# Aedelon/ProteinBERT-PyTorch-Replication

Measured on AMD Instinct MI355X. Metric: sequences/sec (whole node) ProteinBERT pretrain L=512 at 1/2/4/8 MI355X, higher is better.
Workload: dtype bf16; 1 GPU; global_batch=2048, per_gpu_batch=2048, seq_len=512, parallelism=dp1, impl=hip, hip_graph=False

## Files before the change

### proteinbert_pytorch_replication_amd/ops/fused_model.py

```python
from __future__ import annotations

from typing import Dict, Tuple

import torch
import torch.nn.functional as F

from .global_track import FusedGlobalBlockFn, GlobalBlockFn, HeadsLossFn, InputLayerFn, glob_fused_ok, pack_batch
from . import local_track as _lt
from .local_track import CH, EmbedFn, conv_images, embed_tokens, local_block, wgrad_tok_ok
from .paper_track import PaperHeadsLossFn, paper_block, unit_attention_weight


def hip_supported(model) -> Tuple[bool, str]:
    cfg = model.config
    if cfg["local_dim"] != CH:
        return False, f"local_dim={cfg['local_dim']} (HIP kernels are specialised for 128)"
    if cfg["conv_kernel_size"] != 9:
        return False, f"conv_kernel_size={cfg['conv_kernel_size']} (HIP kernels are specialised for 9)"
    if cfg["vocab_size"] > 32:
        return False, "vocab_size > 32"
    if cfg["semantics"] == "paper":
        from .paper_attention import KEY_DIM, VALUE_DIM
        if cfg["key_dim"] != KEY_DIM or cfg["global_dim"] // cfg["num_heads"] != VALUE_DIM:
            return False, (f"paper semantics: the HIP attention core is built for key_dim={KEY_DIM}, "
                           f"value_dim={VALUE_DIM}")
    if (cfg["global_dim"] % 32) != 0:
        return False, "global_dim must be a multiple of 32"
    return True, ""


def _check(model) -> None:
    ok, why = hip_supported(model)
    if not ok:
        raise NotImplementedError(f"HIP backend: unsupported configuration: {why}")


def fused_encode(model, tokens: torch.Tensor, annotations: torch.Tensor,
                 return_bf16: bool = False, cp=None):
    _check(model)
    if cp is None:
        model.check_length(tokens.shape[1])
    else:
        model.check_length(cp.L)
        if tokens.shape[1] != cp.shard_len:
            raise ValueError(f"expected a {cp.shard_len}-residue shard, got {tokens.shape[1]}")
    blocks = list(model.proteinBERT_blocks)
    lin = model.global_linear_layer[0]
    gl0 = blocks[0].global_to_local_linear_layer[0]
    g, g_bf, gb = InputLayerFn.apply(annotations, lin.weight, lin.bias, gl0.weight, gl0.bias)
    paper = model.semantics == "paper"
    emb_w = model.local_embedding.weight
    tok_c = tokens.contiguous()
    fold = (_lt.EMBED_FOLD and cp is None and tokens.device.type == "cuda" and len(blocks) > 0
            and wgrad_tok_ok(tok_c, emb_w, tokens.shape[1], blocks[0].local_narrow_conv_layer[0].weight.shape[2]))
    if fold and not paper and _lt.EMBED_GATHER:
        h = None
    else:
        h = embed_tokens(tok_c, emb_w) if fold else EmbedFn.apply(tokens, emb_w)
    mask = (tokens != 0).contiguous() if paper else None
    items, conv_imgs, glob_imgs = [], [], []
    for i, blk in enumerate(blocks):
        imgs, it = conv_images(blk.local_narrow_conv_layer[0].weight, blk.local_wide_conv_layer[0].weight)
        conv_imgs.append(imgs)
        items += it
        nxt = blocks[i + 1].global_to_local_linear_layer[0] if i + 1 < len(blocks) else None
        if glob_fused_ok(g.shape[1], 0 if nxt is None else nxt.weight.shape[0]):
            ws = [blk.global_linear_layer_1[0].weight, blk.global_linear_layer_2[0].weight,
                  None if nxt is None else nxt.weight]
            imgs = []
            for w in ws:
                if w is None:
                    imgs += [None, None]
                    continue
                o1, o2 = (torch.empty(w.numel(), dtype=torch.bfloat16, device=w.device) for _ in range(2))
                imgs += [o1, o2]
                items.append((1, w.detach(), o1, o2, w.shape[0], w.shape[1]))
            glob_imgs.append(tuple(imgs))
        else:
            glob_imgs.append(None)
    pack_batch(items)
    for i, blk in enumerate(blocks):
        att = blk.global_attention_layer
        if paper:
            first = i == 0 and cp is None
            h, o = paper_block(h, gb, g, blk, mask, conv_imgs[i], tok=tok_c if first else None,
                               emb=emb_w if first else None, emb_grad=fold and i == 0, cp=cp)
            vpart = o.unsqueeze(1)
            wp = unit_attention_weight(att.key_dim, h.device)
        else:
            first = i == 0 and cp is None
            h, vpart = local_block(h, gb, blk, conv_imgs[i], tail=(i == 0), cp=cp,
                                   tok=tok_c if first else None, emb=emb_w if first else None,
                                   emb_grad=fold and i == 0)
            if cp is not None:
                vpart = cp.pool_sum(vpart)
            wp = att.W_parameter
        nxt = blocks[i + 1].global_to_local_linear_layer[0] if i + 1 < len(blocks) else None
        l1, l2 = blk.global_linear_layer_1[0], blk.global_linear_layer_2[0]
        n1, n2 = blk.global_norm_1, blk.global_norm_2
        args = (g, g_bf, vpart, l1.weight, l1.bias, n1.weight, n1.bias, l2.weight, l2.bias, n2.weight, n2.bias,
                wp, None if nxt is None else nxt.weight, None if nxt is None else nxt.bias)
        if glob_imgs[i] is not None:
            g, g_bf, gb = FusedGlobalBlockFn.apply(*args, glob_imgs[i])
        else:
            g, g_bf, gb = GlobalBlockFn.apply(*args)
    if return_bf16:
        return h, g, g_bf
    return h, g


def fused_forward(model, tokens: torch.Tensor, annotations: torch.Tensor):
    h, g = fused_encode(model, tokens, annotations)
    return model.heads_torch(h, g)


def fused_pretrain_loss(model, X: Dict[str, torch.Tensor], Y: Dict[str, torch.Tensor], W: Dict[str, torch.Tensor],
                        return_parts: bool = False, cp=None):
    h, g, g_bf = fused_encode(model, X["local"], X["global"], return_bf16=True, cp=cp)
    if cp is not None:
        W = dict(W, local=W["local"].float() * (cp.shard_len / cp.L))
    lo, go = model.pretraining_local_output[0], model.pretraining_global_output[0]
    fn = PaperHeadsLossFn if model.semantics == "paper" else HeadsLossFn
    total, parts = fn.apply(h, g, g_bf, lo.weight, lo.bias, go.weight, go.bias, Y["local"], Y["global"],
                                     W["local"], W["global"])
    if return_parts:
        return total, parts[0], parts[1]
    return total
```

### proteinbert_pytorch_replication_amd/ops/local_track.py

```python
from __future__ import annotations

import ctypes
import os
from typing import List, Dict, Optional, Tuple

import torch

from . import _lib, streams
from ..train.arena import notify_grads_ready
from ..utils.determinism import fused_deterministic
from .global_track import bf16_of

_P, _I, _F, _L = ctypes.c_void_p, ctypes.c_int, ctypes.c_float, ctypes.c_long

_lib.register("pbx_conv_fwd3x", [_P, _P, _P, _P, _P, _P, _P, _P, _P, _P, _I, _I, _I, _I, _I, _I, _P])
_lib.register("pbx_conv_fwd5x", [_P, _P, _P, _P, _P, _P, _P, _P, _P, _P, _I, _I, _I, _I, _I, _I, _P])
_lib.register("pbx_conv_dgrad4x", [_P, _P, _P, _P, _P, _P, _P, _P, _I, _I, _I, _I, _I, _I, _P])
_lib.register("pbx_wgrad2x", [_P, _P, _P, _P, _P, _P, _P, _P, _P, _I, _I, _I, _I, _I, _I, _I, _P])
_lib.register("pbx_pack_conv_frag", [_P, _P, _P, _I, _P])
_lib.register("pbx_wgrad2", [_P, _P, _P, _P, _P, _P, _P, _P, _P, _I, _I, _I, _I, _I, _P])
_lib.register("pbx_wgrad_tok", [_P, _P, _P, _P, _P, _P, _P, _P, _P, _P, _I, _I, _I, _I, _P, _P, _P, _P, _P])
_lib.register("pbx_ln_linear_fwd", [_P, _P, _I, _I, _P, _P, _P, _P, _P, _P, _P, _I, _I, _F, _P])
_lib.register("pbx_pool_fwd", [_P, _P, _P, _P, _P, _P, _P, _I, _I, _I, _F, _P])
_lib.register("pbx_pool_bwd", [_P, _P, _P, _P, _P, _I, _P, _P, _P, _I, _I, _I, _P])
_lib.register("pbx_ln2_linear_bwd", [_P, _P, _P, _P, _I, _P, _P, _P, _P, _I, _I, _P, _P, _P, _P, _P, _P, _P, _P,
                                     _P, _P, _P, _P, _P, _I, _I, _F, _P, _I, _I, _I, _I, _P])
_lib.register("pbx_ln2_bwd_slab_rows", [_I, _I, _I])
_lib.register("pbx_colsum_add", [_P, _I, _I, _P, _P, _P])
_lib.register("pbx_colsum_add2", [_P, _I, _P, _P, _I, _P, _I, _P])
_lib.register("pbx_ln1_finalize", [_P, _P, _P, _I, _I, _P, _I, _P, _P, _P, _I, _I, _F, _I, _P])
_lib.register("pbx_embed_fwd", [_P, _P, _P, _L, _P])
_lib.register("pbx_embed_bwd", [_P, _P, _P, _L, _I, _P, _P])
_lib.register("pbx_conv_fwd3t", [_P, _P, _P, _P, _P, _P, _P, _P, _P, _P, _P, _I, _I, _I, _I, _P])
_lib.register("pbx_conv_dgrad4f", [_P, _P, _P, _I, _I, _P, _I, _P, _P, _P, _P, _P, _P, _P, _P, _P, _I, _I, _I, _I,
                                    _F, _P])
_lib.register("pbx_embed_dpre", [_P, _P, _P, _P, _P, _P, _P, _L, _I, _P, _P])
_lib.register("pbx_embed_bwd_groups", [_L])

CH = 128
PB = 32
LN_EPS = 1e-5


BM1 = 128
def attn_pool_supported(NJ: int) -> bool:
    return NJ in (256, 512)


def conv_tile(L: int) -> int:
    return BM1


def _p(t: Optional[torch.Tensor]):
    return None if t is None else t.data_ptr()


CONV_FWD5 = os.environ.get("PBX_CONV_FWD", "5") == "5"


def conv_dgrad_fin(dh1, s1, st1, T1, BM1, sums1, TS1, g1, gdn, gdw, wtn, wtw, dx, dpn, dpw, dgb, B, L, KS, dil,
                   stream):
    _lib.call("pbx_conv_dgrad4f", dh1.data_ptr(), s1.data_ptr(), st1.data_ptr(), T1, BM1, sums1.data_ptr(),
              TS1, g1.data_ptr(), gdn.data_ptr(), gdw.data_ptr(), wtn.data_ptr(), wtw.data_ptr(),
              dx.data_ptr(), dpn.data_ptr(), dpw.data_ptr(), dgb.data_ptr(), B, L, KS, dil, LN_EPS, stream)


def conv_fwd(x, wpn, wpw, bn, bw, gb, pre_n, pre_w, s1, stats, B, L, KS, dil, stream, xlo: int = 0,
             xhi: int = 0) -> None:
    name = "pbx_conv_fwd5x" if (CONV_FWD5 and KS == 9 and dil == 5) else "pbx_conv_fwd3x"
    _lib.call(name, x.data_ptr(), wpn.data_ptr(), wpw.data_ptr(), bn.data_ptr(), bw.data_ptr(),
              gb.data_ptr(), _p(pre_n), _p(pre_w), s1.data_ptr(), stats.data_ptr(), B, L, KS, dil, xlo, xhi, stream)


def conv_dgrad(ds1, pre_n, pre_w, wtn, wtw, dx, dpn, dpw, B, L, KS, dil, stream, ilo: int = 0, ihi: int = 0) -> None:
    _lib.call("pbx_conv_dgrad4x", ds1.data_ptr(), pre_n.data_ptr(), pre_w.data_ptr(), wtn.data_ptr(),
              wtw.data_ptr(), dx.data_ptr(), dpn.data_ptr(), dpw.data_ptr(), B, L, KS, dil, ilo, ihi, stream)


_DWL_SLAB: Dict[int, torch.Tensor] = {}


def dwl_slab(dev: torch.device) -> Tuple[Optional[int], int]:
    idx = dev.index if dev.index is not None else torch.cuda.current_device()
    s = _DWL_SLAB.get(idx)
    rows = 2 * _num_cus(dev)
    if s is None:
        s = torch.empty(rows * (CH * CH + CH), dtype=torch.float32, device=dev)
        _DWL_SLAB[idx] = s
    return s.data_ptr(), rows


def _num_cus(dev: torch.device) -> int:
    return torch.cuda.get_device_properties(dev).multi_processor_count


def pack_conv(w: torch.Tensor) -> Tuple[torch.Tensor, torch.Tensor]:
    KS = w.shape[2]
    wp = torch.empty((KS, CH, CH), dtype=torch.bfloat16, device=w.device)
    wt = torch.empty_like(wp)
    _lib.call("pbx_pack_conv_frag", w.detach().contiguous().data_ptr(), wp.data_ptr(), wt.data_ptr(), KS,
              _lib.stream_ptr(w.device))
    return wp, wt


def _grad_dst(p: torch.Tensor, shape) -> Tuple[torch.Tensor, bool]:
    g = getattr(p, "grad", None) if getattr(p, "_pbx_arena", False) else None
    if g is not None and g.is_contiguous() and g.dtype == torch.float32 and tuple(g.shape) == tuple(shape):
        return g, True
    return torch.zeros(shape, dtype=torch.float32, device=p.device), False


WGRAD_TAIL_FULL = True
LN2_LATE_FOLD = True
DGRAD_FIN = True
INPUT_BWD_EARLY = True


WGRAD_CU_EIGHTHS = 8


def _wgrad(dy0: torch.Tensor, dy1: Optional[torch.Tensor], x: torch.Tensor, KS: int, dil: int, nconv: int,
           B: int, L: int, outs, full_chip: bool = False, xlo: int = 0, xhi: int = 0):
    dev = x.device
    ntiles = B * ((L + 127) // 128)
    R = max(8, (WGRAD_CU_EIGHTHS * _num_cus(dev) // (16 * nconv)) // 8 * 8)
    if full_chip:
        R = max(8, (_num_cus(dev) // (2 * nconv)) // 8 * 8)
    R = min(R, ntiles)
    slab = torch.empty((R, nconv, KS, CH, CH), dtype=torch.float32, device=dev)
    bslab = torch.empty((R, nconv, CH), dtype=torch.float32, device=dev)
    (dw0, db0) = outs[0]
    (dw1, db1) = outs[1] if nconv > 1 else (None, None)
    if xlo or xhi:
        _lib.call("pbx_wgrad2x", dy0.data_ptr(), _p(dy1), x.data_ptr(), slab.data_ptr(), bslab.data_ptr(),
                  dw0.data_ptr(), _p(dw1), db0.data_ptr(), _p(db1), B, L, dil, nconv, R, xlo, xhi, _lib.stream_ptr(dev))
    else:
        _lib.call("pbx_wgrad2", dy0.data_ptr(), _p(dy1), x.data_ptr(), slab.data_ptr(), bslab.data_ptr(),
                  dw0.data_ptr(), _p(dw1), db0.data_ptr(), _p(db1), B, L, dil, nconv, R, _lib.stream_ptr(dev))
    return [slab, bslab]


WGRAD_TOK = True
EMBED_FOLD = True
EMBED_GATHER = True


def wgrad_tok_ok(tok: Optional[torch.Tensor], emb: Optional[torch.Tensor], L: int, KS: int) -> bool:
    return (WGRAD_TOK and tok is not None and emb is not None and KS == 9 and L % 2 == 0
            and emb.shape[0] <= 32 and emb.shape[1] == CH and tok.dtype == torch.int64 and tok.is_contiguous())


def _wgrad_tok(dy0: torch.Tensor, dy1: torch.Tensor, tok: torch.Tensor, emb: torch.Tensor, dil: int, B: int, L: int,
               outs, demb=None):
    dev = dy0.device
    V = emb.shape[0]
    R = _lib.lib().pbx_wgrad_tok_rows(B, L)
    slab = torch.empty((R, 2, 9, V, CH), dtype=torch.float32, device=dev)
    S = torch.empty((2, 9, V, CH), dtype=torch.float32, device=dev)
    e = emb.detach().float().contiguous()
    (dw0, db0), (dw1, db1) = outs
    w0 = w1 = dE = dEslab = None
    if demb is not None:
        w0, w1 = (w.detach().float().contiguous() for w in demb[:2])
        dE = demb[2]
        dEslab = torch.empty((2 * CH, V, CH), dtype=torch.float32, device=dev)
    _lib.call("pbx_wgrad_tok", tok.data_ptr(), dy0.data_ptr(), dy1.data_ptr(), e.data_ptr(), slab.data_ptr(),
              S.data_ptr(), dw0.data_ptr(), dw1.data_ptr(), db0.data_ptr(), db1.data_ptr(), B, L, dil, V,
              _p(w0), _p(w1), _p(dE), _p(dEslab), _lib.stream_ptr(dev))
    return [slab, S, e, w0, w1, dEslab]


def embed_fold_bwd(tok, emb, ds1, gdn, gdw, dpn, dpw, wn, ww, stream):
    B, L = tok.shape
    dE, direct = _grad_dst(emb, emb.shape)
    slab = None
    if fused_deterministic():
        slab = torch.empty((_lib.lib().pbx_embed_bwd_groups(B * L), emb.shape[0], CH), dtype=torch.float32,
                           device=ds1.device)
    _lib.call("pbx_embed_dpre", tok.data_ptr(), ds1.data_ptr(), gdn.data_ptr(), gdw.data_ptr(), dpn.data_ptr(),
              dpw.data_ptr(), dE.data_ptr(), B * L, emb.shape[0], _p(slab), stream)
    return (wn, ww, dE), direct


class LocalBlockFn(torch.autograd.Function):

    @staticmethod
    def forward(ctx, x, gb, wn, bn, ww, bw, g1, be1, wl, bl, g2, be2, wv_bf16, dil: int, packed=None,
                tail: bool = False, cp=None, tok=None, emb=None, emb_grad: bool = False):
        params = (wn, bn, ww, bw, g1, be1, wl, bl, g2, be2)
        ctx.cp = cp
        if cp is not None:
            g1, be1, g2, be2 = (cp.rows(t) for t in (g1, be1, g2, be2))
        if x is None:
            if not (emb_grad and tok is not None and emb is not None and cp is None):
                raise ValueError("x may be None only for the folded first block (emb_grad with tok / emb)")
            B, L = tok.shape
            xt = torch.empty((B, L, CH), dtype=torch.bfloat16, device=tok.device)
        else:
            B, L, C = x.shape
            assert C == CH and x.dtype == torch.bfloat16 and x.is_contiguous()
            xt = x
        NJ = wv_bf16.shape[0]
        if not attn_pool_supported(NJ):
            raise NotImplementedError(f"HIP attention pool: H * value_dim = {NJ} (kernels built for 256 / 512)")
        KS = wn.shape[2]
        dev = xt.device
        stream = _lib.stream_ptr(dev)
        T1 = (L + BM1 - 1) // BM1
        T2 = (L + PB - 1) // PB
        if packed is not None:
            wpn, wtn, wpw, wtw = packed
        else:
            wpn, wtn = pack_conv(wn)
            wpw, wtw = pack_conv(ww)
        wl_b = bf16_of(wl)
        need_bwd = any(ctx.needs_input_grad)
        pre_n = torch.empty_like(xt) if need_bwd else None
        pre_w = torch.empty_like(xt) if need_bwd else None
        s1 = torch.empty_like(xt)
        st1 = torch.empty((B, T1, 2), dtype=torch.float32, device=dev)
        gb = gb.detach().float().contiguous()
        if x is None:
            x_ext, hlo = None, 0
            emb_b = bf16_of(emb)
            _lib.call("pbx_conv_fwd3t", tok.data_ptr(), emb_b.data_ptr(), wpn.data_ptr(), wpw.data_ptr(),
                      bn.data_ptr(), bw.data_ptr(), gb.data_ptr(), _p(pre_n), _p(pre_w), s1.data_ptr(),
                      st1.data_ptr(), B, L, KS, dil, stream)
        elif cp is None:
            x_ext, hlo = x, 0
            conv_fwd(x, wpn, wpw, bn, bw, gb, pre_n, pre_w, s1, st1, B, L, KS, dil, stream)
        else:
            x_ext, hlo = cp.halo_rows(x), cp.halo
            conv_fwd(x_ext, wpn, wpw, bn, bw, gb, pre_n, pre_w, s1, st1, B, L, KS, dil, stream, hlo, hlo)
            cp.fix_stats(st1, BM1)
        pre_l = torch.empty_like(xt) if need_bwd else None
        s2 = torch.empty_like(xt)
        st2 = torch.empty((B, T2, 2), dtype=torch.float32, device=dev)
        _lib.call("pbx_ln_linear_fwd", s1.data_ptr(), st1.data_ptr(), T1, BM1, g1.data_ptr(), be1.data_ptr(),
                  wl_b.data_ptr(), bl.data_ptr(), _p(pre_l), s2.data_ptr(), st2.data_ptr(), B, L, LN_EPS, stream)
        if cp is not None:
            cp.fix_stats(st2, PB)
        h2 = torch.empty_like(xt)
        TV = (L + 31) // 32
        vpart = torch.empty((B, TV, NJ), dtype=torch.float32, device=dev)
        _lib.call("pbx_pool_fwd", s2.data_ptr(), st2.data_ptr(), g2.data_ptr(), be2.data_ptr(), wv_bf16.data_ptr(),
                  h2.data_ptr(), vpart.data_ptr(), B, L, NJ, LN_EPS, stream)
        ctx.save_for_backward(x_ext, pre_n, pre_w, s1, st1, pre_l, s2, st2, h2, wtn, wtw, wl_b, wv_bf16, g1, be1, g2,
                              be2)
        ctx.hlo = hlo
        ctx.tok = (tok, emb) if cp is None and wgrad_tok_ok(tok, emb, L, KS) else None
        ctx.emb_grad = bool(emb_grad)
        if ctx.emb_grad and (ctx.tok is None or (x is not None and x.requires_grad)):
            raise ValueError("emb_grad needs a token-embedding input without autograd history (wgrad_tok_ok)")
        ctx.meta = (B, L, KS, dil, T1, T2, NJ)
        ctx.tail = bool(tail) and WGRAD_TAIL_FULL
        ctx.set_materialize_grads(False)
        ctx.params = params
        return h2, vpart

    @staticmethod
    def backward(ctx, dh2, dvpart):
        streams.wait_ready(dvpart, dh2)
        (x_ext, pre_n, pre_w, s1, st1, pre_l, s2, st2, h2, wtn, wtw, wl_b, wv_bf16, g1, be1, g2,
         be2) = ctx.saved_tensors
        cp, hlo = ctx.cp, ctx.hlo
        x = s1
        B, L, KS, dil, T1, T2, NJ = ctx.meta
        dev = x.device
        stream = _lib.stream_ptr(dev)
        params = ctx.params
        dsts = [_grad_dst(p, p.shape) for p in params]
        (dwn, _), (dbn, _), (dww, _), (dbw, _), (dg1, _), (dbe1, _), (dwl, _), (dbl, _), (dg2, _), (dbe2, _) = dsts
        if cp is not None:
            dg1, dbe1, dg2, dbe2 = (cp.rows(t) for t in (dg1, dbe1, dg2, dbe2))
        dh2 = None if dh2 is None else dh2.to(torch.bfloat16).contiguous()
        TA = (L + 31) // 32
        if dvpart is None:
            dv, dv_tiles = torch.zeros((B, NJ), dtype=torch.float32, device=dev), 1
        elif dvpart.dim() == 3 and (dvpart.shape[1] == 1 or dvpart.stride(1) == 0):
            dv, dv_tiles = dvpart[:, 0, :].float().contiguous(), 1
        else:
            dv, dv_tiles = dvpart.float().contiguous(), TA
        dh2t = torch.empty_like(x)
        sums2 = torch.empty((B, TA, 2), dtype=torch.float32, device=dev)
        consts = torch.empty((B, 8), dtype=torch.float32, device=dev)
        dgb = torch.empty((B, CH), dtype=torch.float32, device=dev)
        _lib.call("pbx_pool_bwd", h2.data_ptr(), g2.data_ptr(), be2.data_ptr(), _p(dh2), dv.data_ptr(), dv_tiles,
                  wv_bf16.data_ptr(), dh2t.data_ptr(), sums2.data_ptr(), B, L, NJ, stream)
        if cp is not None:
            cp.fix_sums(sums2)
        dh1 = torch.empty_like(x)
        TS1 = (L + 1) // 2
        sums1 = torch.empty((B, TS1, 2), dtype=torch.float32, device=dev)
        det = int(fused_deterministic())
        late_fold = LN2_LATE_FOLD and streams.ENABLED and dev.type == "cuda" and dsts[6][1] and dsts[7][1]
        if late_fold:
            rows = _lib.lib().pbx_ln2_bwd_slab_rows(B, L, det)
            fslab = torch.empty(rows * (CH * CH + CH), dtype=torch.float32, device=dev)
            slab_args = (fslab.data_ptr(), rows)
        else:
            slab_args = dwl_slab(dev)
        _lib.call("pbx_ln2_linear_bwd", dh2t.data_ptr(), s2.data_ptr(), st2.data_ptr(), sums2.data_ptr(), TA,
                  g2.data_ptr(), pre_l.data_ptr(), s1.data_ptr(), st1.data_ptr(), T1, BM1, g1.data_ptr(),
                  be1.data_ptr(), wl_b.data_ptr(), consts.data_ptr(), dh1.data_ptr(), sums1.data_ptr(),
                  dg2.data_ptr(), dbe2.data_ptr(), dg1.data_ptr(), dbe1.data_ptr(), dwl.data_ptr(), dbl.data_ptr(),
                  dgb.data_ptr(), B, L, LN_EPS, *slab_args, det, int(not late_fold), 0, stream)
        if late_fold:
            def fold(slab=fslab, rows=rows, dwl=dwl, dbl=dbl):
                st = _lib.stream_ptr(dev)
                _lib.call("pbx_colsum_add2", slab.data_ptr(), CH * CH, dwl.data_ptr(), slab[rows * CH * CH:].data_ptr(),
                          CH, dbl.data_ptr(), rows, st)
            streams.launch(dev, fold, keep=[fslab], name="wgrad")
        dx = None if ctx.emb_grad else torch.empty_like(x)
        dpn = torch.empty_like(x)
        dpw = torch.empty_like(x)
        if cp is not None:
            cp.fix_sums(sums1)
        fin = (DGRAD_FIN and cp is None and not ctx.emb_grad and KS == 9 and dev.type == "cuda"
               and not fused_deterministic())

        def dgb_ready():
            if ctx.tail and INPUT_BWD_EARLY and streams.ENABLED and dev.type == "cuda":
                streams.fork(dev, "ann")

        if not fin:
            ds1 = torch.empty_like(x)
            _lib.call("pbx_ln1_finalize", dh1.data_ptr(), s1.data_ptr(), st1.data_ptr(), T1, BM1, sums1.data_ptr(),
                      TS1, g1.data_ptr(), ds1.data_ptr(), dgb.data_ptr(), B, L, LN_EPS, int(fused_deterministic()),
                      stream)
            if cp is not None:
                cp.all_reduce_(dgb)
            dgb_ready()
        demb = None
        if fin:
            conv_dgrad_fin(dh1, s1, st1, T1, BM1, sums1, TS1, g1, pre_n, pre_w, wtn, wtw, dx, dpn, dpw, dgb, B, L,
                           KS, dil, stream)
            dgb_ready()
        elif ctx.emb_grad:
            demb, dE_direct = embed_fold_bwd(*ctx.tok, ds1, pre_n, pre_w, dpn, dpw, params[0], params[2], stream)
            dE = demb[2]
        elif cp is None:
            conv_dgrad(ds1, pre_n, pre_w, wtn, wtw, dx, dpn, dpw, B, L, KS, dil, stream)
        else:
            conv_dgrad(*cp.halo_rows_many(ds1, pre_n, pre_w), wtn, wtw, dx, dpn, dpw, B, L,
                       KS, dil, stream, hlo, hlo)
        if ctx.tok is not None:
            tok, emb = ctx.tok
            wg = lambda: _wgrad_tok(dpn, dpw, tok, emb, dil, B, L, [(dwn, dbn), (dww, dbw)], demb)
            keep = [dpn, dpw, tok] + ([demb[2]] if demb is not None else [])
        else:
            wg = lambda: _wgrad(dpn, dpw, x_ext, KS, dil, 2, B, L, [(dwn, dbn), (dww, dbw)],
                                ctx.tail and streams.ENABLED, hlo, hlo)
            keep = [dpn, dpw, x_ext]
        direct = [p for p, (_, d) in zip(params, dsts) if d]
        if demb is not None and dE_direct:
            direct.append(ctx.tok[1])
        if all(dsts[i][1] for i in (0, 1, 2, 3)) and (demb is None or dE_direct) and streams.ENABLED:
            streams.launch(dev, wg, keep=keep, name="wgrad")
        else:
            wg()
        if direct:
            notify_grads_ready(direct)
        pgrads = [None if d else g for (g, d) in dsts]
        gemb = dE if demb is not None and not dE_direct else None
        return (dx, dgb, *pgrads, None, None, None, None, None, None, gemb, None)


def embed_tokens(tokens: torch.Tensor, weight: torch.Tensor) -> torch.Tensor:
    B, L = tokens.shape
    tok = tokens.contiguous()
    out = torch.empty((B, L, weight.shape[1]), dtype=torch.bfloat16, device=tokens.device)
    _lib.call("pbx_embed_fwd", tok.data_ptr(), weight.detach().contiguous().data_ptr(), out.data_ptr(), B * L,
              _lib.stream_ptr(tokens.device))
    return out


class EmbedFn(torch.autograd.Function):

    @staticmethod
    def forward(ctx, tokens, weight):
        B, L = tokens.shape
        V, C = weight.shape
        assert C == CH and V <= 32
        tok = tokens.contiguous()
        out = torch.empty((B, L, C), dtype=torch.bfloat16, device=tokens.device)
        _lib.call("pbx_embed_fwd", tok.data_ptr(), weight.detach().contiguous().data_ptr(), out.data_ptr(), B * L,
                  _lib.stream_ptr(tokens.device))
        ctx.save_for_backward(tok)
        ctx.V = V
        return out

    @staticmethod
    def backward(ctx, dout):
        (tok,) = ctx.saved_tensors
        dE = torch.zeros((ctx.V, CH), dtype=torch.float32, device=tok.device)
        d = dout.to(torch.bfloat16).contiguous()
        slab = None
        if fused_deterministic():
            g = _lib.lib().pbx_embed_bwd_groups(tok.numel())
            slab = torch.empty((g, ctx.V, CH), dtype=torch.float32, device=tok.device)
        _lib.call("pbx_embed_bwd", tok.data_ptr(), d.data_ptr(), dE.data_ptr(), tok.numel(), ctx.V, _lib.ptr(slab),
                  _lib.stream_ptr(tok.device))
        return None, dE


def _wv_bf16(att) -> torch.Tensor:
    Wv = att.Wv
    if isinstance(Wv, torch.nn.Parameter) and Wv.requires_grad:
        return att.value_weight_cat().t().to(torch.bfloat16).contiguous()
    key = (Wv.data_ptr(), Wv._version, Wv.device)
    cached = getattr(att, "_pbx_wv_cache", None)
    if cached is None or cached[0] != key:
        cached = (key, att.value_weight_cat().t().to(torch.bfloat16).contiguous())
        att._pbx_wv_cache = cached
    return cached[1]


def conv_images(wn: torch.Tensor, ww: torch.Tensor):
    KS = wn.shape[2]
    imgs = tuple(torch.empty((KS, CH, CH), dtype=torch.bfloat16, device=wn.device) for _ in range(4))
    return imgs, [(0, wn.detach(), imgs[0], imgs[1], KS, 0), (0, ww.detach(), imgs[2], imgs[3], KS, 0)]


def local_block(x: torch.Tensor, gb: torch.Tensor, blk, packed=None, tail: bool = False,
                cp=None, tok=None, emb=None, emb_grad: bool = False) -> Tuple[torch.Tensor, torch.Tensor]:
    att = blk.global_attention_layer
    wv = _wv_bf16(att)
    nc = blk.local_narrow_conv_layer[0]
    wc = blk.local_wide_conv_layer[0]
    return LocalBlockFn.apply(x, gb, nc.weight, nc.bias, wc.weight, wc.bias, blk.local_norm_1.weight,
                              blk.local_norm_1.bias, blk.local_linear_layer[0].weight, blk.local_linear_layer[0].bias,
                              blk.local_norm_2.weight, blk.local_norm_2.bias, wv, blk.wide_conv_dilation, packed,
                              tail, cp, tok, emb, emb_grad)
```

Measured before the change: 106,600 sequences/s.

## Compute first-block convolutions from per-token lookup tables instead of MFMA conv

The first local block's input is a token embedding, so each conv tap's output depends only on the token id. This precomputes per-(kernel tap, vocab id) fp32 tables of weight·embedding and replaces the first block's narrow and wide convolution GEMMs with LDS table lookups and sums, fused with bias, GELU, residual and LayerNorm stats. Stats granularity changes to 4-row tiles, so bm1 is threaded through the LN kernels. It adds a small table-building kernel each step and large LDS use per workgroup, and accumulating in fp32 from tables slightly changes rounding versus the bf16 MFMA path.

```diff
diff --git a/proteinbert_pytorch_replication_amd/ops/csrc/conv_tok.hip b/proteinbert_pytorch_replication_amd/ops/csrc/conv_tok.hip
--- /dev/null
+++ b/proteinbert_pytorch_replication_amd/ops/csrc/conv_tok.hip
@@ -0,0 +1,242 @@
+#include "mfma.h"
+
+using namespace pbx;
+typedef unsigned short bf16_t;
+
+namespace {
+constexpr int CH = 128;
+constexpr int HC = 64;
+constexpr int BM = 128;
+constexpr int KS = 9;
+constexpr int MAXHALO = 20;
+constexpr int NT = 1024;
+constexpr int WP = BM / (NT / 64);
+constexpr int WTOK = WP + 2 * MAXHALO;
+
+__global__ void __launch_bounds__(256) conv_tok_tables_kernel(const bf16x8* __restrict__ fwn,
+                                                              const bf16x8* __restrict__ fww,
+                                                              const bf16_t* __restrict__ emb, float* __restrict__ tab,
+                                                              int V) {
+  const int R = V + 1;
+  const int idx = blockIdx.x * 256 + threadIdx.x;
+  if (idx >= 2 * KS * R * CH) return;
+  const int co = idx & 127;
+  int r = idx >> 7;
+  const int v = r % R;
+  r /= R;
+  const int k = r % KS, c = r / KS;
+  float acc = 0.f;
+  if (v < V) {
+    const bf16x8* fw = c ? fww : fwn;
+#pragma unroll
+    for (int q = 0; q < 16; ++q) {
+      const uint4 wq = *reinterpret_cast<const uint4*>(fw + (size_t)(((k * 8 + (q >> 1)) * 4 + (co >> 5)) * 64 +
+                                                                     (co & 31) + 32 * (q & 1)));
+      const uint4 eq = *reinterpret_cast<const uint4*>(emb + (size_t)v * CH + q * 8);
+      float wv[8], ev[8];
+      unpack8(wq, wv);
+      unpack8(eq, ev);
+#pragma unroll
+      for (int j = 0; j < 8; ++j) acc = fmaf(wv[j], ev[j], acc);
+    }
+  }
+  tab[((size_t)(((co >> 6) * 2 + c) * KS + k) * R + v) * HC + (co & 63)] = acc;
+}
+
+__device__ __forceinline__ f32x2 lo2(const float4& v) { return (f32x2){v.x, v.y}; }
+__device__ __forceinline__ f32x2 hi2(const float4& v) { return (f32x2){v.z, v.w}; }
+
+__device__ __forceinline__ unsigned pk2(const f32x2& v) {
+  typedef __bf16 bf16x2 __attribute__((ext_vector_type(2)));
+  return __builtin_bit_cast(unsigned, __builtin_convertvector(v, bf16x2));
+}
+__device__ __forceinline__ f32x2 unpk2(unsigned q) {
+  return (f32x2){__uint_as_float(q << 16), __uint_as_float(q & 0xffff0000u)};
+}
+
+template <bool STORE, int DIL>
+__global__ void __launch_bounds__(NT) conv_fwd_tok_kernel(
+    const long long* __restrict__ tok, const bf16_t* __restrict__ emb, const float* __restrict__ tab,
+    const float* __restrict__ bn, const float* __restrict__ bw, const float* __restrict__ gb,
+    bf16_t* __restrict__ pre_n, bf16_t* __restrict__ pre_w, bf16_t* __restrict__ s1, float* __restrict__ stats,
+    int B, int L, int dil_arg, int V) {
+  extern __shared__ __attribute__((aligned(16))) unsigned char smem[];
+  const int R = V + 1;
+  const int RS = R * 256;
+  unsigned char* tabs = smem;
+  unsigned char* xe = tabs + 2 * KS * RS;
+  const int tid = threadIdx.x, lane = tid & 63, w = tid >> 6;
+  float* bias = reinterpret_cast<float*>(xe + R * 128);
+  int* wt = reinterpret_cast<int*>(bias + 2 * HC) + w * WTOK;
+  const int hf = blockIdx.x & 1;
+  const int T = L / BM, NU = B * T;
+  const int nwg = gridDim.x >> 1;
+  const int dil = DIL ? DIL : dil_arg;
+  const int halo = 4 * dil;
+  const int c4 = tid & 15, q = lane >> 4;
+  const int wtoks = WP + 2 * halo;
+  const int ch0 = hf * HC + c4 * 4;
+
+  auto tok_off = [&](int u, int i) {
+    const int b = u / T, pos = (u - b * T) * BM + w * WP - halo + i;
+    int v = V;
+    if (pos >= 0 && pos < L) {
+      const long long t = tok[(size_t)b * L + pos];
+      v = (t >= 0 && t < V) ? (int)t : V;
+    }
+    return v << 8;
+  };
+
+  int u = blockIdx.x >> 1;
+  {
+    const uint4* src = reinterpret_cast<const uint4*>(tab + (size_t)hf * 2 * KS * R * HC);
+    stage_chunks(
+        2 * KS * R * 16, [&](int idx) { return src[idx]; },
+        [&](int idx, uint4 v) { *reinterpret_cast<uint4*>(tabs + idx * 16) = v; });
+    for (int idx = tid; idx < R * 8; idx += NT) {
+      const int v = idx >> 3;
+      const uint4 xr = v < V ? *reinterpret_cast<const uint4*>(emb + (size_t)v * CH + hf * HC + (idx & 7) * 8)
+                             : make_uint4(0u, 0u, 0u, 0u);
+      *reinterpret_cast<uint4*>(xe + idx * 16) = xr;
+    }
+  }
+  int tcur = u < NU && lane < wtoks ? tok_off(u, lane) : 0;
+  if (tid < 2 * HC) bias[tid] = tid < HC ? bn[hf * HC + tid] : bw[hf * HC + tid - HC];
+  float4 gbv = u < NU ? *reinterpret_cast<const float4*>(gb + (size_t)(u / T) * CH + ch0) : make_float4(0.f, 0.f, 0.f, 0.f);
+  __syncthreads();
+
+  for (; u < NU; u += nwg) {
+    const int b = u / T, t = u - b * T;
+    const int un = u + nwg;
+    if (lane < wtoks) wt[lane] = tcur;
+    __builtin_amdgcn_fence(__ATOMIC_SEQ_CST, "wavefront");
+    __builtin_amdgcn_wave_barrier();
+    float4 gbn = gbv;
+    if (un < NU && lane < wtoks) tcur = tok_off(un, lane);
+    if (un < NU) gbn = *reinterpret_cast<const float4*>(gb + (size_t)(un / T) * CH + ch0);
+    const f32x2 gbp[2] = {lo2(gbv), hi2(gbv)};
+    f32x2 sum2 = {0.f, 0.f}, sq2 = {0.f, 0.f};
+#pragma unroll 1
+    for (int ps = 0; ps < 2; ++ps) {
+      const int p = w * WP + ps * 4 + q;
+      const int* to = wt + halo + ps * 4 + q;
+      const unsigned char* tb = tabs + c4 * 16;
+      int on[KS], ow[KS];
+#pragma unroll
+      for (int k = 0; k < KS; ++k) {
+        on[k] = to[k - 4];
+        ow[k] = to[(k - 4) * dil];
+      }
+      float4 rn[KS], rw[KS];
+#pragma unroll
+      for (int k = 0; k < KS; ++k) rn[k] = *reinterpret_cast<const float4*>(tb + k * RS + on[k]);
+#pragma unroll
+      for (int k = 0; k < KS; ++k) rw[k] = *reinterpret_cast<const float4*>(tb + (KS + k) * RS + ow[k]);
+      __builtin_amdgcn_sched_barrier(0);
+      f32x2 an[2] = {lo2(rn[0]), hi2(rn[0])}, aw[2] = {lo2(rw[0]), hi2(rw[0])};
+#pragma unroll
+      for (int k = 1; k < KS; ++k) {
+        an[0] += lo2(rn[k]);
+        an[1] += hi2(rn[k]);
+      }
+#pragma unroll
+      for (int k = 1; k < KS; ++k) {
+        aw[0] += lo2(rw[k]);
+        aw[1] += hi2(rw[k]);
+      }
+      const uint2 xq = *reinterpret_cast<const uint2*>(xe + (to[0] >> 1) + c4 * 8);
+      const float4 bnv = *reinterpret_cast<const float4*>(bias + c4 * 4);
+      const float4 bwv = *reinterpret_cast<const float4*>(bias + HC + c4 * 4);
+      an[0] += lo2(bnv); an[1] += hi2(bnv);
+      aw[0] += lo2(bwv); aw[1] += hi2(bwv);
+      const f32x2 gi[4] = {unpk2(pk2(an[0])), unpk2(pk2(an[1])), unpk2(pk2(aw[0])), unpk2(pk2(aw[1]))};
+      const f32x2 xv[2] = {unpk2(xq.x), unpk2(xq.y)};
+      f32x2 go[4];
+      const unsigned off = (((unsigned)b * L + t * BM + p) * CH + ch0) * 2;
+      if constexpr (STORE) {
+        f32x2 gd[4];
+        gelu_n<4, 2>(gi, go, gd);
+        *reinterpret_cast<uint2*>(reinterpret_cast<unsigned char*>(pre_n) + off) = make_uint2(pk2(gd[0]), pk2(gd[1]));
+        *reinterpret_cast<uint2*>(reinterpret_cast<unsigned char*>(pre_w) + off) = make_uint2(pk2(gd[2]), pk2(gd[3]));
+      } else {
+        gelu_n<4, 0>(gi, go, nullptr);
+      }
+      uint2 oq;
+      {
+#pragma clang fp contract(off)
+        oq.x = pk2(xv[0] + go[0] + go[2] + gbp[0]);
+        oq.y = pk2(xv[1] + go[1] + go[3] + gbp[1]);
+      }
+      *reinterpret_cast<uint2*>(reinterpret_cast<unsigned char*>(s1) + off) = oq;
+      const f32x2 r0 = unpk2(oq.x), r1 = unpk2(oq.y);
+      sum2 += r0;
+      sum2 += r1;
+      sq2 = __builtin_elementwise_fma(r0, r0, sq2);
+      sq2 = __builtin_elementwise_fma(r1, r1, sq2);
+    }
+    {
+      const float sa = wave_reduce_sum(sum2.x + sum2.y), sq = wave_reduce_sum(sq2.x + sq2.y);
+      if (lane == 0) {
+        const float n = (float)(WP * HC), m = sa / n;
+        float* dst = stats + (((size_t)b * T + t) * (2 * NT / 64) + hf * (NT / 64) + w) * 2;
+        dst[0] = m;
+        dst[1] = fmaxf(sq - sa * m, 0.f);
+      }
+    }
+    gbv = gbn;
+    __builtin_amdgcn_fence(__ATOMIC_SEQ_CST, "wavefront");
+    __builtin_amdgcn_wave_barrier();
+  }
+}
+
+int tok_lds(int V) { return 2 * KS * (V + 1) * 256 + (V + 1) * 128 + 2 * HC * 4 + (NT / 64) * WTOK * 4; }
+
+int num_cus() {
+  static int cus = 0;
+  if (cus == 0) {
+    int dev = 0, n = 0;
+    if (hipGetDevice(&dev) != hipSuccess ||
+        hipDeviceGetAttribute(&n, hipDeviceAttributeMultiprocessorCount, dev) != hipSuccess || n < 2)
+      n = 256;
+    cus = n;
+  }
+  return cus;
+}
+}
+
+PBX_EXPORT int pbx_conv_fwd_tok_ok(int B, int L, int KS_, int dil, int V) {
+  return B >= 1 && L >= BM && L % BM == 0 && KS_ == KS && dil >= 1 && 4 * dil <= MAXHALO && V >= 1 && V <= 32 &&
+         tok_lds(V) <= 163840 && (long long)B * L < (1ll << 24);
+}
+
+PBX_EXPORT int pbx_conv_tok_tables(const void* fwn, const void* fww, const void* emb, float* tab, int V,
+                                   hipStream_t st) {
+  if (V < 1 || V > 32) return (int)hipErrorInvalidValue;
+  const int n = 2 * KS * (V + 1) * CH;
+  hipLaunchKernelGGL(conv_tok_tables_kernel, dim3((n + 255) / 256), dim3(256), 0, st, (const bf16x8*)fwn,
+                     (const bf16x8*)fww, (const bf16_t*)emb, tab, V);
+  return pbx_launch_status();
+}
+
+PBX_EXPORT int pbx_conv_fwd_tok(const long long* tok, const void* emb, const float* tab, const float* bn,
+                                const float* bw, const float* gb, void* pre_n, void* pre_w, void* s1, float* stats,
+                                int B, int L, int KS_, int dil, int V, hipStream_t st) {
+  if (!pbx_conv_fwd_tok_ok(B, L, KS_, dil, V) || tok == nullptr || emb == nullptr || tab == nullptr || gb == nullptr ||
+      (pre_n == nullptr) != (pre_w == nullptr))
+    return (int)hipErrorInvalidValue;
+  static bool attrs_set = false;
+  if (!attrs_set) {
+    for (const void* k : {(const void*)conv_fwd_tok_kernel<true, 5>, (const void*)conv_fwd_tok_kernel<false, 5>,
+                          (const void*)conv_fwd_tok_kernel<true, 0>, (const void*)conv_fwd_tok_kernel<false, 0>})
+      (void)hipFuncSetAttribute(k, hipFuncAttributeMaxDynamicSharedMemorySize, 163840);
+    attrs_set = true;
+  }
+  const int NU = B * (L / BM);
+  int grid = num_cus() & ~1;
+  if (grid > 2 * NU) grid = 2 * NU;
+  const auto kern = dil == 5 ? (pre_n != nullptr ? conv_fwd_tok_kernel<true, 5> : conv_fwd_tok_kernel<false, 5>)
+                             : (pre_n != nullptr ? conv_fwd_tok_kernel<true, 0> : conv_fwd_tok_kernel<false, 0>);
+  hipLaunchKernelGGL(kern, dim3(grid), dim3(NT), tok_lds(V), st, tok, (const bf16_t*)emb, tab, bn, bw, gb,
+                     (bf16_t*)pre_n, (bf16_t*)pre_w, (bf16_t*)s1, stats, B, L, dil, V);
+  return pbx_launch_status();
+}
diff --git a/proteinbert_pytorch_replication_amd/ops/fused_model.py b/proteinbert_pytorch_replication_amd/ops/fused_model.py
--- a/proteinbert_pytorch_replication_amd/ops/fused_model.py
+++ b/proteinbert_pytorch_replication_amd/ops/fused_model.py
@@ -5,7 +5,8 @@
 import torch
 import torch.nn.functional as F
 
-from .global_track import FusedGlobalBlockFn, GlobalBlockFn, HeadsLossFn, InputLayerFn, glob_fused_ok, pack_batch
+from .global_track import (FusedGlobalBlockFn, GlobalBlockFn, HeadsLossFn, InputLayerFn, bf16_of, glob_fused_ok,
+                           pack_batch)
 from . import local_track as _lt
 from .local_track import CH, EmbedFn, conv_images, embed_tokens, local_block, wgrad_tok_ok
 from .paper_track import PaperHeadsLossFn, paper_block, unit_attention_weight
@@ -79,6 +80,12 @@
         else:
             glob_imgs.append(None)
     pack_batch(items)
+    tok_tab = None
+    if h is None:
+        nc0 = blocks[0].local_narrow_conv_layer[0]
+        if _lt.conv_tok_ok(tok_c.shape[0], tok_c.shape[1], nc0.weight.shape[2], blocks[0].wide_conv_dilation,
+                           emb_w.shape[0]):
+            tok_tab = _lt.conv_tok_tables(conv_imgs[0][0], conv_imgs[0][2], bf16_of(emb_w))
     for i, blk in enumerate(blocks):
         att = blk.global_attention_layer
         if paper:
@@ -91,7 +98,7 @@
             first = i == 0 and cp is None
             h, vpart = local_block(h, gb, blk, conv_imgs[i], tail=(i == 0), cp=cp,
                                    tok=tok_c if first else None, emb=emb_w if first else None,
-                                   emb_grad=fold and i == 0)
+                                   emb_grad=fold and i == 0, tok_tab=tok_tab if i == 0 else None)
             if cp is not None:
                 vpart = cp.pool_sum(vpart)
             wp = att.W_parameter
diff --git a/proteinbert_pytorch_replication_amd/ops/local_track.py b/proteinbert_pytorch_replication_amd/ops/local_track.py
--- a/proteinbert_pytorch_replication_amd/ops/local_track.py
+++ b/proteinbert_pytorch_replication_amd/ops/local_track.py
@@ -36,6 +36,9 @@
                                     _F, _P])
 _lib.register("pbx_embed_dpre", [_P, _P, _P, _P, _P, _P, _P, _L, _I, _P, _P])
 _lib.register("pbx_embed_bwd_groups", [_L])
+_lib.register("pbx_conv_fwd_tok_ok", [_I, _I, _I, _I, _I])
+_lib.register("pbx_conv_tok_tables", [_P, _P, _P, _P, _I, _P])
+_lib.register("pbx_conv_fwd_tok", [_P, _P, _P, _P, _P, _P, _P, _P, _P, _P, _I, _I, _I, _I, _I, _P])
 
 CH = 128
 PB = 32
@@ -145,6 +148,41 @@
 EMBED_GATHER = True
 
 
+CONV_TOK = os.environ.get("PBX_CONV_TOK", "1") == "1"
+
+
+def conv_tok_ok(B: int, L: int, KS: int, dil: int, V: int) -> bool:
+    return CONV_TOK and bool(_lib.lib().pbx_conv_fwd_tok_ok(B, L, KS, dil, V))
+
+
+def conv_tok_tables(wpn: torch.Tensor, wpw: torch.Tensor, emb_b: torch.Tensor) -> torch.Tensor:
+    V = emb_b.shape[0]
+    tab = torch.empty((2, 2, 9, V + 1, CH // 2), dtype=torch.float32, device=emb_b.device)
+    _lib.call("pbx_conv_tok_tables", wpn.data_ptr(), wpw.data_ptr(), emb_b.data_ptr(), tab.data_ptr(), V,
+              _lib.stream_ptr(emb_b.device))
+    return tab
+
+
+def conv_fwd_first(tok, emb_b, wpn, wpw, bn, bw, gb, pre_n, pre_w, s1, KS, dil, stream, tok_tab=None):
+    B, L = tok.shape
+    V = emb_b.shape[0]
+    if conv_tok_ok(B, L, KS, dil, V):
+        T1, bm1 = L // 4, 4
+        st1 = torch.empty((B, T1, 2), dtype=torch.float32, device=tok.device)
+        if tok_tab is None:
+            tok_tab = conv_tok_tables(wpn, wpw, emb_b)
+        _lib.call("pbx_conv_fwd_tok", tok.data_ptr(), emb_b.data_ptr(), tok_tab.data_ptr(), bn.data_ptr(),
+                  bw.data_ptr(), gb.data_ptr(), _p(pre_n), _p(pre_w), s1.data_ptr(), st1.data_ptr(), B, L, KS, dil, V,
+                  stream)
+    else:
+        T1, bm1 = (L + BM1 - 1) // BM1, BM1
+        st1 = torch.empty((B, T1, 2), dtype=torch.float32, device=tok.device)
+        _lib.call("pbx_conv_fwd3t", tok.data_ptr(), emb_b.data_ptr(), wpn.data_ptr(), wpw.data_ptr(), bn.data_ptr(),
+                  bw.data_ptr(), gb.data_ptr(), _p(pre_n), _p(pre_w), s1.data_ptr(), st1.data_ptr(), B, L, KS, dil,
+                  stream)
+    return st1, T1, bm1
+
+
 def wgrad_tok_ok(tok: Optional[torch.Tensor], emb: Optional[torch.Tensor], L: int, KS: int) -> bool:
     return (WGRAD_TOK and tok is not None and emb is not None and KS == 9 and L % 2 == 0
             and emb.shape[0] <= 32 and emb.shape[1] == CH and tok.dtype == torch.int64 and tok.is_contiguous())
@@ -186,7 +224,7 @@
 
     @staticmethod
     def forward(ctx, x, gb, wn, bn, ww, bw, g1, be1, wl, bl, g2, be2, wv_bf16, dil: int, packed=None,
-                tail: bool = False, cp=None, tok=None, emb=None, emb_grad: bool = False):
+                tail: bool = False, cp=None, tok=None, emb=None, emb_grad: bool = False, tok_tab=None):
         params = (wn, bn, ww, bw, g1, be1, wl, bl, g2, be2)
         ctx.cp = cp
         if cp is not None:
@@ -206,7 +244,7 @@
         KS = wn.shape[2]
         dev = xt.device
         stream = _lib.stream_ptr(dev)
-        T1 = (L + BM1 - 1) // BM1
+        T1, bm1 = (L + BM1 - 1) // BM1, BM1
         T2 = (L + PB - 1) // PB
         if packed is not None:
             wpn, wtn, wpw, wtw = packed
@@ -218,25 +256,28 @@
         pre_n = torch.empty_like(xt) if need_bwd else None
         pre_w = torch.empty_like(xt) if need_bwd else None
         s1 = torch.empty_like(xt)
-        st1 = torch.empty((B, T1, 2), dtype=torch.float32, device=dev)
         gb = gb.detach().float().contiguous()
-        if x is None:
-            x_ext, hlo = None, 0
+        from_tok = x is None or (cp is None and tok is not None and emb is not None and tok.dtype == torch.int64
+                                 and tok.is_contiguous() and tuple(tok.shape) == (B, L) and emb.shape[1] == CH
+                                 and conv_tok_ok(B, L, KS, dil, emb.shape[0]))
+        if from_tok:
+            x_ext, hlo = x, 0
             emb_b = bf16_of(emb)
-            _lib.call("pbx_conv_fwd3t", tok.data_ptr(), emb_b.data_ptr(), wpn.data_ptr(), wpw.data_ptr(),
-                      bn.data_ptr(), bw.data_ptr(), gb.data_ptr(), _p(pre_n), _p(pre_w), s1.data_ptr(),
-                      st1.data_ptr(), B, L, KS, dil, stream)
+            st1, T1, bm1 = conv_fwd_first(tok, emb_b, wpn, wpw, bn, bw, gb, pre_n, pre_w, s1, KS, dil, stream,
+                                          tok_tab)
         elif cp is None:
             x_ext, hlo = x, 0
+            st1 = torch.empty((B, T1, 2), dtype=torch.float32, device=dev)
             conv_fwd(x, wpn, wpw, bn, bw, gb, pre_n, pre_w, s1, st1, B, L, KS, dil, stream)
         else:
             x_ext, hlo = cp.halo_rows(x), cp.halo
+            st1 = torch.empty((B, T1, 2), dtype=torch.float32, device=dev)
             conv_fwd(x_ext, wpn, wpw, bn, bw, gb, pre_n, pre_w, s1, st1, B, L, KS, dil, stream, hlo, hlo)
             cp.fix_stats(st1, BM1)
         pre_l = torch.empty_like(xt) if need_bwd else None
         s2 = torch.empty_like(xt)
         st2 = torch.empty((B, T2, 2), dtype=torch.float32, device=dev)
-        _lib.call("pbx_ln_linear_fwd", s1.data_ptr(), st1.data_ptr(), T1, BM1, g1.data_ptr(), be1.data_ptr(),
+        _lib.call("pbx_ln_linear_fwd", s1.data_ptr(), st1.data_ptr(), T1, bm1, g1.data_ptr(), be1.data_ptr(),
                   wl_b.data_ptr(), bl.data_ptr(), _p(pre_l), s2.data_ptr(), st2.data_ptr(), B, L, LN_EPS, stream)
         if cp is not None:
             cp.fix_stats(st2, PB)
@@ -253,6 +294,7 @@
         if ctx.emb_grad and (ctx.tok is None or (x is not None and x.requires_grad)):
             raise ValueError("emb_grad needs a token-embedding input without autograd history (wgrad_tok_ok)")
         ctx.meta = (B, L, KS, dil, T1, T2, NJ)
+        ctx.bm1 = bm1
         ctx.tail = bool(tail) and WGRAD_TAIL_FULL
         ctx.set_materialize_grads(False)
         ctx.params = params
@@ -266,6 +308,7 @@
         cp, hlo = ctx.cp, ctx.hlo
         x = s1
         B, L, KS, dil, T1, T2, NJ = ctx.meta
+        bm1 = ctx.bm1
         dev = x.device
         stream = _lib.stream_ptr(dev)
         params = ctx.params
@@ -301,7 +344,7 @@
         else:
             slab_args = dwl_slab(dev)
         _lib.call("pbx_ln2_linear_bwd", dh2t.data_ptr(), s2.data_ptr(), st2.data_ptr(), sums2.data_ptr(), TA,
-                  g2.data_ptr(), pre_l.data_ptr(), s1.data_ptr(), st1.data_ptr(), T1, BM1, g1.data_ptr(),
+                  g2.data_ptr(), pre_l.data_ptr(), s1.data_ptr(), st1.data_ptr(), T1, bm1, g1.data_ptr(),
                   be1.data_ptr(), wl_b.data_ptr(), consts.data_ptr(), dh1.data_ptr(), sums1.data_ptr(),
                   dg2.data_ptr(), dbe2.data_ptr(), dg1.data_ptr(), dbe1.data_ptr(), dwl.data_ptr(), dbl.data_ptr(),
                   dgb.data_ptr(), B, L, LN_EPS, *slab_args, det, int(not late_fold), 0, stream)
@@ -325,7 +368,7 @@
 
         if not fin:
             ds1 = torch.empty_like(x)
-            _lib.call("pbx_ln1_finalize", dh1.data_ptr(), s1.data_ptr(), st1.data_ptr(), T1, BM1, sums1.data_ptr(),
+            _lib.call("pbx_ln1_finalize", dh1.data_ptr(), s1.data_ptr(), st1.data_ptr(), T1, bm1, sums1.data_ptr(),
                       TS1, g1.data_ptr(), ds1.data_ptr(), dgb.data_ptr(), B, L, LN_EPS, int(fused_deterministic()),
                       stream)
             if cp is not None:
@@ -333,7 +376,7 @@
             dgb_ready()
         demb = None
         if fin:
-            conv_dgrad_fin(dh1, s1, st1, T1, BM1, sums1, TS1, g1, pre_n, pre_w, wtn, wtw, dx, dpn, dpw, dgb, B, L,
+            conv_dgrad_fin(dh1, s1, st1, T1, bm1, sums1, TS1, g1, pre_n, pre_w, wtn, wtw, dx, dpn, dpw, dgb, B, L,
                            KS, dil, stream)
             dgb_ready()
         elif ctx.emb_grad:
@@ -363,7 +406,7 @@
             notify_grads_ready(direct)
         pgrads = [None if d else g for (g, d) in dsts]
         gemb = dE if demb is not None and not dE_direct else None
-        return (dx, dgb, *pgrads, None, None, None, None, None, None, gemb, None)
+        return (dx, dgb, *pgrads, None, None, None, None, None, None, gemb, None, None)
 
 
 def embed_tokens(tokens: torch.Tensor, weight: torch.Tensor) -> torch.Tensor:
@@ -423,7 +466,7 @@
 
 
 def local_block(x: torch.Tensor, gb: torch.Tensor, blk, packed=None, tail: bool = False,
-                cp=None, tok=None, emb=None, emb_grad: bool = False) -> Tuple[torch.Tensor, torch.Tensor]:
+                cp=None, tok=None, emb=None, emb_grad: bool = False, tok_tab=None) -> Tuple[torch.Tensor, torch.Tensor]:
     att = blk.global_attention_layer
     wv = _wv_bf16(att)
     nc = blk.local_narrow_conv_layer[0]
@@ -431,4 +474,4 @@
     return LocalBlockFn.apply(x, gb, nc.weight, nc.bias, wc.weight, wc.bias, blk.local_norm_1.weight,
                               blk.local_norm_1.bias, blk.local_linear_layer[0].weight, blk.local_linear_layer[0].bias,
                               blk.local_norm_2.weight, blk.local_norm_2.bias, wv, blk.wide_conv_dilation, packed,
-                              tail, cp, tok, emb, emb_grad)
+                              tail, cp, tok, emb, emb_grad, tok_tab)
```

After: 107,900 sequences/s (median of 6 runs). 1.2% higher.
